# CPCLAB-UNIPI/MPC-code

Measured on AMD Instinct MI355X. Metric: closed-loop MPC steps/sec over batch, LMPC-CSTR N=50, higher is better.
Workload: dtype f64

## Files before the change

mpc-code_amd/csrc/mpc_amd.hip:

```cpp
#include "../../include/mpc_amd.h"
#include "mpc_device.hpp"
#include "mpc_tp.hpp"
#include "mpc_wave.hpp"
#include "mpc_soft.hpp"
#ifdef MPC_NL_PLANT_HEADER
#include MPC_NL_PLANT_HEADER
#endif

#include <hip/hip_runtime.h>
#include "mpc_comm.hpp"

#include <cmath>
#include <cstdint>
#include <cstdio>
#include <cstring>
#include <string>
#include <vector>

using namespace mpc;

#ifndef MPC_PART2
extern "C" const char *mpc_last_error(void) { return g_err; }
#endif

// ... 924 lines not shown
        X[j].put(X0);
    }
    MPC_STAMP_INIT
    int redo = 0;
    for (int k = 0; k < a.nsteps; k++) {
        unsigned bq = (unsigned)b;
        asm volatile("" : "+v"(bq));
        if (redo == 0) {
        if constexpr (RT::fits) {
            const int b16 = lane >> 4, r16 = lane & 15, b16c = b16 < NI ? b16 : 0;
            const unsigned bi = (unsigned)(blockIdx.x * NI + b16c);
            const bool inst16 = b16 < NI && (int)bi < a.B;
            double *const kq = keep + b16c * KEEP;
            if (inst16) {
                if (a.XP && r16 < NXP) (a.XP + (size_t)((size_t)k * NXP + r16) * Bs)[bi] = kq[KC::K_X + r16];
                if (a.XHAT && r16 < NX) (a.XHAT + (size_t)((size_t)k * NX + r16) * Bs)[bi] = kq[KC::K_XH + r16];
            }
            double xi_old = 0.0, xi_new = 0.0;
            if (P.estimator != MPC_EST_NONE)
                kalman_row16<NX, NY, ND, NXP, NU>(P, r16, b16 < NI, kq, KC::K_X, KC::K_XH, KC::K_P, a.pyp + k * NY, tab, T + b16c * RT::XCH, xi_old, xi_new);
            if (inst16 && a.DHAT && r16 >= NX && r16 < NE) (a.DHAT + (size_t)((size_t)k * ND + (r16 - NX)) * Bs)[bi] = xi_new;
            double delta = row16_max(r16 < NE ? fabs(xi_new - xi_old) : 0.0);
            __syncthreads();
            if (Cfg::RZ * NI * LD < 4 * RT::XCH) { for (int i = lane; i < NI * LD; i += 64) T[Cfg::RZ * NI * LD + i] = 0.0; }
            double dh[NDD], usv[NU];
            MPC_UNROLL for (int i = 0; i < ND; i++) dh[i] = kq[KC::K_DH + i];
            MPC_UNROLL for (int i = 0; i < NU; i++) usv[i] = kq[KC::K_US + i];
            int it_ss; double vrow;
            const int st_ss = target_row16<NX, NU, NY, ND, NGS, NHS>(P, r16, tab, a.usp + k * NU, a.ysp + k * NY, dh, usv, kq + KC::K_TW, twv + b16c, inst16, vrow, it_ss);
            const bool trow = r16 < NX + NU && b16 < NI;
            const double prev = trow ? kq[KC::K_XS + r16] : 0.0;
            const double tnew = (st_ss != kInfeasible && trow) ? vrow : prev;
            delta = dmax(delta, row16_max(fabs(tnew - prev)));
            if (trow) kq[KC::K_XS + r16] = tnew;
            if (inst16) {
                if (a.XS && r16 < NX) (a.XS + (size_t)((size_t)k * NX + r16) * Bs)[bi] = tnew;
                if (a.US && r16 >= NX && trow) (a.US + (size_t)((size_t)k * NU + (r16 - NX)) * Bs)[bi] = tnew;
                if (a.st_dyn && r16 == 0) { (a.st_ss + (size_t)k * Bs)[bi] = st_ss; (a.it_ss + (size_t)k * Bs)[bi] = it_ss; }
            }
            if (r16 == 0 && b16 < NI) outv[b16c * Cfg::OUT] = delta;
            __syncthreads();
        }
        if (valid) {
            double xh[NX], dh[NDD], u[NU], xs[NX], us[NU], delta = 0.0;
            MPC_UNROLL for (int i = 0; i < NX; i++) { xh[i] = kp[KC::K_XH + i]; xs[i] = kp[KC::K_XS + i]; }
            MPC_UNROLL for (int i = 0; i < ND; i++) dh[i] = kp[KC::K_DH + i];
            MPC_UNROLL for (int i = 0; i < NU; i++) { u[i] = kp[KC::K_U + i]; us[i] = kp[KC::K_US + i]; }
            if constexpr (RT::fits) delta = outv[lane * Cfg::OUT];
            else {
                double x[NXP];
                double xh_pred[NX], dh_prev[NDD], xs_prev[NX], us_prev[NU];
                MPC_UNROLL for (int i = 0; i < NXP; i++) x[i] = kp[KC::K_X + i];
                MPC_UNROLL for (int i = 0; i < NX; i++) { xh[i] = kp[KC::K_XH + i]; xs[i] = kp[KC::K_XS + i]; xh_pred[i] = xh[i]; xs_prev[i] = xs[i]; }
                MPC_UNROLL for (int i = 0; i < ND; i++) { dh[i] = kp[KC::K_DH + i]; dh_prev[i] = dh[i]; }
                MPC_UNROLL for (int i = 0; i < NU; i++) { u[i] = kp[KC::K_U + i]; us[i] = kp[KC::K_US + i]; us_prev[i] = us[i]; }
                if (a.XP) { MPC_UNROLL for (int i = 0; i < NXP; i++) (a.XP + (size_t)((size_t)k * NXP + i) * Bs)[bq] = x[i]; }
                if (a.XHAT) { MPC_UNROLL for (int i = 0; i < NX; i++) (a.XHAT + (size_t)((size_t)k * NX + i) * Bs)[bq] = xh[i]; }
                if (P.estimator != MPC_EST_NONE) {
                    double xi[NE], innov[NY];
                    MPC_UNROLL for (int i = 0; i < NX; i++) xi[i] = xh[i];
                    MPC_UNROLL for (int i = 0; i < ND; i++) xi[NX + i] = dh[i];
                    MPC_UNROLL for (int i = 0; i < NY; i++) {
                        double yh = P.fyc[i], yy = a.pyp[k * NY + i];
                        MPC_UNROLL for (int j = 0; j < NE; j++) yh += P.Ca[i][j] * xi[j];
// ... 32 lines not shown
            if (a.YS) {
                MPC_UNROLL for (int i = 0; i < NY; i++) {
                    double v = P.fyc[i];
                    MPC_UNROLL for (int j = 0; j < NX; j++) v += P.Cm[i][j] * xs[j];
                    MPC_UNROLL for (int j = 0; j < ND; j++) v += P.Cd[i][j] * dh[j];
                    (a.YS + (size_t)((size_t)k * NY + i) * Bs)[bq] = v;
                }
            }
            OcpInst<NS, NU> qi;
            build_inst<NX, NU, NY, ND, DU, NG>(P, xh, xs, us, dh, u, qi);
            const bool warm = wsv[lane] != 0 && delta <= kWsDelta && !P.no_warm;
            double *qd = q + lane * Cfg::QN;
            MPC_UNROLL for (int i = 0; i < NS; i++) { qd[i] = qi.z0[i]; qd[NS + i] = qi.zr[i]; qd[2 * NS + i] = qi.c[i]; qd[3 * NS + i] = qi.zlo_m[i]; qd[4 * NS + i] = qi.zhi_m[i]; qd[Cfg::QZN + i] = qi.zrN[i]; }
            MPC_UNROLL for (int i = 0; i < NU; i++) { qd[5 * NS + i] = qi.ur[i]; qd[5 * NS + NU + i] = qi.us[i]; }
            qd[5 * NS + 2 * NU] = delta;
            iflag[lane] = kWvValid | (qi.ok0 ? kWvOk0 : 0) | (warm ? kWvWarm : 0);
            itacc[lane] = 0;
            MPC_UNROLL for (int i = 0; i < NX; i++) { kp[KC::K_XH + i] = xh[i]; kp[KC::K_XS + i] = xs[i]; }
            MPC_UNROLL for (int i = 0; i < ND; i++) kp[KC::K_DH + i] = dh[i];
            MPC_UNROLL for (int i = 0; i < NU; i++) kp[KC::K_US + i] = us[i];
        } else if (lane < NI) iflag[lane] = 0;
        __syncthreads();
        }
        MPC_TSTAMP(0);
        wv_solve<NS, NU, DU, NC, MASKED, NI>(P, T, q, iflag, X, S, P.max_iter);
        MPC_STAMP_RESET
        if (lane == 0) {
            MPC_UNROLL for (int j = 0; j < NI; j++) {
                MPC_UNROLL for (int i = 0; i < NU; i++) outv[j * Cfg::OUT + i] = a_get(X[j].u[i]);
                MPC_UNROLL for (int i = 0; i < NS; i++) outv[j * Cfg::OUT + NU + i] = a_get(X[j].z[i]);
            }
        }
        if (P.term_cons && lane == P.N - 1) {
            MPC_UNROLL for (int j = 0; j < NI; j++) {
                double v = 0.0, c[NX];
                MPC_UNROLL for (int i = 0; i < NX; i++) { const double zr = q[j * Cfg::QN + NS + i]; c[i] = a_get(X[j].z[i]) - zr; v = dmax(v, fabs(c[i]) * frcp(dmax(1.0, fabs(zr)))); }
                outv[j * Cfg::OUT + NU + NS] = v;
                const int f = iflag[j];
                const bool again = redo < 2 && (f & kWvValid) && (f & kWvOk0) && S[j].status != kInfeasible && v > 1e-11 && v <= 1e-4;
                if (again) { MPC_UNROLL for (int i = 0; i < NX; i++) q[j * Cfg::QN + Cfg::QZN + i] -= c[i]; q[j * Cfg::QN + 5 * NS + 2 * NU] = v; }
                aimv[j] = again ? 1 : 0;
            }
        }
        __syncthreads();
        if (P.term_cons && redo < 2) {
            int any = 0;
            MPC_UNROLL for (int j = 0; j < NI; j++) any |= aimv[j];
// ... 1377 lines not shown
```

mpc-code_amd/csrc/mpc_tp.hpp:

```cpp
#pragma once
#include "mpc_device.hpp"

#ifdef MPC_STAMPS
#define MPC_TSTAMP(slot) do { const unsigned long long t_ = __builtin_amdgcn_s_memtime(); __builtin_amdgcn_s_waitcnt(0xC07F); \
    if (threadIdx.x == 0 && threadIdx.y == 0) mpc_stamp_buf[(blockIdx.x & 4095) * 8 + (slot)] += t_ - stamp_prev_; stamp_prev_ = t_; } while (0)
#else
#define MPC_TSTAMP(slot) do { } while (0)
#endif
#ifdef MPC_STAMPS_FINE
#define MPC_TSTAMP_IT(slot) MPC_TSTAMP(3)
#define MPC_TSTAMP_FINE(slot) MPC_TSTAMP(slot)
#else
#define MPC_TSTAMP_IT(slot) MPC_TSTAMP(slot)
#define MPC_TSTAMP_FINE(slot) do { } while (0)
#endif

namespace mpc {

template <int NS, int NU, int NC, int NW, int IPW, int XKEEP = 0>
struct TpCfg {
    static constexpr int NI = NW * IPW;
    static constexpr int NV = NS + NU, NKF = NU * NS, NLI = NU * (NU + 1) / 2;
    static constexpr int RA = 0, RA_SZ = (NC > NKF + NLI ? NC : NKF + NLI);
    static constexpr int RG = RA_SZ, RK = RG + NV, ROWS = RK + NU;
    static constexpr int LD = 65;
    static constexpr int T_DOUBLES = ROWS * NI * LD;
    static constexpr int QN = 5 * NS + 2 * NU + 1;
    static constexpr int ST_SL = 0, ST_SH = NC, ST_LL = 2 * NC, ST_LH = 3 * NC, ST_DV = 4 * NC, ST_U = 5 * NC, ST_Z = 5 * NC + NU, ROWS_ST = 5 * NC + NV;
    static constexpr int KEEP_MAX = 2 * NU + 3 * (NS + NU + 8) + XKEEP;
    static constexpr size_t lds_bytes() { return sizeof(double) * (T_DOUBLES + NI * QN + NI * 4 + NI * KEEP_MAX) + sizeof(int) * (4 * NI + 4); }
};

template <int CTRL, int ROW_MASK>
__device__ __forceinline__ double dpp_move(double old, double v)
{
    union { double d; int i[2]; } a, o, r; a.d = v; o.d = old;
    r.i[0] = __builtin_amdgcn_update_dpp(o.i[0], a.i[0], CTRL, ROW_MASK, 0xF, false);
// ... 622 lines not shown
```

mpc-code_amd/csrc/mpc_wave.hpp:

```cpp
#pragma once
#include "mpc_device.hpp"
#include "mpc_tp.hpp"

namespace mpc {

#ifdef MPC_WV_GENERIC_TILES
constexpr bool kWvGenericTiles = true;
#else
constexpr bool kWvGenericTiles = false;
#endif

template <int NS, int NU, int NC, int NI_>
struct WvCfg {
    static constexpr int NI = NI_;
    static constexpr int NV = NS + NU, NKF = NU * NS, NLI = NU * (NU + 1) / 2;
    static constexpr int RA = 0, RA_SZ = (NC > NKF + NLI ? NC : NKF + NLI);
    static constexpr int RG = RA_SZ, RK = RG + NV, RZ = RK + NU, ROWS = RZ + 1;
    __host__ __device__ static constexpr int ld(int N) { return (N + 1) | 1; }
    static constexpr int GUARD = 8;
    __host__ __device__ static constexpr int t_doubles(int N) { return GUARD + ROWS * NI * ld(N); }
    static constexpr int RL_A = ROWS, RL_B = RL_A + NS * NS, RL_C = RL_B + NS * NU, ROWS_LTV = RL_C + NS;
    __host__ __device__ static constexpr int t_doubles_ltv(int N) { return GUARD + ROWS_LTV * NI * ld(N); }
    static constexpr int QZN = 5 * NS + 2 * NU + 1;
    static constexpr int QN = QZN + NS;
// ... 20 lines not shown
    return u.d;
}
template <int NS, int NU, int NC>
struct WvIterA {
    AReg2 sl[NC], sh[NC], ll[NC], lh[NC], u[NU], z[NS];
    __device__ __forceinline__ void get(WvIter<NS, NU, NC> &X) const
    {
        MPC_UNROLL for (int i = 0; i < NC; i++) { X.sl[i] = a_get(sl[i]); X.sh[i] = a_get(sh[i]); X.ll[i] = a_get(ll[i]); X.lh[i] = a_get(lh[i]); }
        MPC_UNROLL for (int i = 0; i < NU; i++) X.u[i] = a_get(u[i]);
        MPC_UNROLL for (int i = 0; i < NS; i++) X.z[i] = a_get(z[i]);
    }
    __device__ __forceinline__ void put(const WvIter<NS, NU, NC> &X)
    {
        MPC_UNROLL for (int i = 0; i < NC; i++) { a_put(sl[i], X.sl[i]); a_put(sh[i], X.sh[i]); a_put(ll[i], X.ll[i]); a_put(lh[i], X.lh[i]); }
        MPC_UNROLL for (int i = 0; i < NU; i++) a_put(u[i], X.u[i]);
        MPC_UNROLL for (int i = 0; i < NS; i++) a_put(z[i], X.z[i]);
    }
};

struct WvInst { double mu, mu_sum, sm, inv_ncon, gscale, res_s, res_p; int stall, iters, status; bool on, warm, keep_u; };

enum : int { kWvOk0 = 1, kWvWarm = 2, kWvValid = 4, kWvKeepU = 8, kWvNoShift = 16 };

__device__ __forceinline__ double row16_sum(double v)
{
    v += dpp_move<0xB1, 0xF>(0.0, v);
    v += dpp_move<0x4E, 0xF>(0.0, v);
    v += dpp_move<0x141, 0xF>(0.0, v);
    v += dpp_move<0x140, 0xF>(0.0, v);
    return v;
}
__device__ __forceinline__ double row16_max(double v)
{
    v = dmax(v, dpp_move<0xB1, 0xF>(v, v));
    v = dmax(v, dpp_move<0x4E, 0xF>(v, v));
    v = dmax(v, dpp_move<0x141, 0xF>(v, v));
    v = dmax(v, dpp_move<0x140, 0xF>(v, v));
    return v;
}

template <int NS, int NU, bool HASM, int NC, bool MASKED, int NI, class PT, bool LTV = false, bool PAIR = false>
__device__ __forceinline__ void wv_solve(const PT &P, double *T, const double *q, const int *iflag,
                                         WvIterA<NS, NU, NC> (&X)[PAIR ? NI / 2 : NI], WvInst (&S)[PAIR ? NI / 2 : NI], int max_iter)
{
    static_assert(!LTV || (NS <= 4 && !HASM), "time-varying stage matrices: one 4 x 4 tile per state matrix, no cross term");
    using Cfg = WvCfg<NS, NU, NC, NI>;
    using Iter = WvIter<NS, NU, NC>;
    constexpr int NV = Cfg::NV, NKF = Cfg::NKF, NLI = Cfg::NLI, RA = Cfg::RA, RG = Cfg::RG, RK = Cfg::RK;
    static_assert(NS <= 8 && NU <= 2 && NI >= 1 && NI <= 4, "stage state <= 8 (2 x 2 tiles of 4 x 4), nu <= 2 (closed-form inverse of Lambda); at most four instances per product");
    static_assert(!PAIR || NI % 2 == 0, "pairs of instances");
    constexpr int NJ = PAIR ? NI / 2 : NI;
    const int lane = threadIdx.x, N = P.N, LD = Cfg::ld(N);
    const int k = PAIR ? (lane & 31) : lane;
    const int hsel = PAIR ? (lane >> 5) : 0;
    auto ji = [&](int j) -> int { return PAIR ? 2 * j + hsel : j; };
    const bool blk_on = k < N, last = k == N - 1;
    auto tk = [&](int row, int j) -> double & { return T[(row * NI + ji(j)) * LD + k]; };
    auto un = [](double v) -> double { return PAIR ? v : uni(v); };
    auto rsum = [](double v) -> double { return PAIR ? half_sum(v) : wave_sum(v); };
    auto rmax = [](double v) -> double { return PAIR ? half_max(v) : wave_max(v); };
    MPC_STAMP_INIT

    auto launder = [](const PT &Pin) -> const PT & { const PT *pp = &Pin; asm volatile("" : "+s"(pp)); return *pp; };
    struct Bnd { double lo[NC], hi[NC]; bool fl[NC], fh[NC]; };
    auto bounds = [&](const PT &Pl, int j, Bnd &Bd) {
        const double *qd = q + ji(j) * Cfg::QN;
        MPC_UNROLL for (int i = 0; i < NC; i++) {
            const double zlm = i >= NU ? qd[3 * NS + (i >= NU ? i - NU : 0)] : 0.0, zhm = i >= NU ? qd[4 * NS + (i >= NU ? i - NU : 0)] : 0.0;
            const double lm = i < NU ? Pl.ulo[i < NU ? i : 0] : zlm, hm = i < NU ? Pl.uhi[i < NU ? i : 0] : zhm;
            const double le = i < NU ? Pl.ulo[i < NU ? i : 0] : Pl.zlo_e[i >= NU ? i - NU : 0], he = i < NU ? Pl.uhi[i < NU ? i : 0] : Pl.zhi_e[i >= NU ? i - NU : 0];
            const double lo = last ? le : lm, hi = last ? he : hm;
            Bd.fl[i] = MASKED ? fin(lo) : true; Bd.fh[i] = MASKED ? fin(hi) : true;
            Bd.lo[i] = Bd.fl[i] ? lo : 0.0; Bd.hi[i] = Bd.fh[i] ? hi : 0.0;
        }
    };
    auto gradient = [&](const PT &Pl, int j, const Iter &Xj, double (&gu)[NU], double (&gz)[NS]) {
        const double *qd = q + ji(j) * Cfg::QN;
        double dz1[NS], du[NU];
        const double *qz = qd + (last ? Cfg::QZN : NS);
        MPC_UNROLL for (int i = 0; i < NS; i++) dz1[i] = Xj.z[i] - qz[i];
        MPC_UNROLL for (int i = 0; i < NU; i++) du[i] = Xj.u[i] - qd[5 * NS + i];
        MPC_UNROLL for (int i = 0; i < NS; i++) {
            double a = (NU + i < NC) ? Xj.lh[NU + i < NC ? NU + i : 0] - Xj.ll[NU + i < NC ? NU + i : 0] : 0.0;
// ... 14 lines not shown
        }
    };
    auto phase_a = [&](const PT &Pl, int j, WvInst &Sj, const Iter &Xj, int it) {
        Bnd Bd; bounds(Pl, j, Bd);
        double mu_p = 0.0, resp_p = 0.0, cres_p = 0.0, lmax_p = 0.0, hb[NC];
        MPC_UNROLL for (int i = 0; i < NC; i++) {
            const double v = i < NU ? Xj.u[i < NU ? i : 0] : Xj.z[i >= NU ? i - NU : 0];
            const double rh = Bd.fh[i] ? v + Xj.sh[i] - Bd.hi[i] : 0.0, rl = Bd.fl[i] ? v - Xj.sl[i] - Bd.lo[i] : 0.0;
            const double isl = frcp(Xj.sl[i]), ish = frcp(Xj.sh[i]);
            mu_p += Xj.sl[i] * Xj.ll[i] + Xj.sh[i] * Xj.lh[i];
            if (blk_on) tk(RA + i, j) = Xj.ll[i] * isl + Xj.lh[i] * ish;
            hb[i] = Xj.lh[i] * (rh * ish - 1.0) + Xj.ll[i] * (rl * isl + 1.0);
            resp_p = dmax(resp_p, dmax(fabs(rl), fabs(rh)));
            cres_p = dmax(cres_p, dmax(comp_measure(Xj.sl[i], Xj.ll[i]), comp_measure(Xj.sh[i], Xj.lh[i])));
            lmax_p = dmax(lmax_p, dmax(Xj.ll[i], Xj.lh[i]));
        }
        double gu[NU], gz[NS], pi[NS];
        gradient(Pl, j, Xj, gu, gz);
        if (blk_on) {
            MPC_UNROLL for (int i = 0; i < NU; i++) tk(RG + i, j) = gu[i] + hb[i];
            MPC_UNROLL for (int i = 0; i < NS; i++) tk(RG + NU + i, j) = gz[i] + (NU + i < NC ? hb[NU + i < NC ? NU + i : 0] : 0.0);
        }
        MPC_UNROLL for (int i = 0; i < NS; i++) pi[i] = blk_on ? gz[i] : 0.0;
        Sj.mu_sum = rsum(blk_on ? mu_p : 0.0);
        const double res_p = rmax(blk_on ? resp_p : 0.0), cres = rmax(blk_on ? cres_p : 0.0), lmax = rmax(blk_on ? lmax_p : 0.0);
        const bool ok_cp = (cres <= 1.0) && (res_p <= kTolFeas);
        double rs_p = 0.0;
        if (LTV) {
            if (it == 0 || ok_cp) {
                double An[NS][NS], g0[NS];
                const int kn = k + 1 < N ? k + 1 : (N > 0 ? N - 1 : 0);
                const bool upd = k + 1 < N;
                MPC_UNROLL for (int i = 0; i < NS; i++) { g0[i] = pi[i]; MPC_UNROLL for (int l = 0; l < NS; l++) { const double v = T[((Cfg::RL_A + i * NS + l) * NI + ji(j)) * LD + kn]; An[i][l] = upd ? v : 0.0; } }
                for (int s = N - 2; s >= 0; s--) {
                    double t[NS];
                    MPC_UNROLL for (int i = 0; i < NS; i++) { const double v = wave_dn1(pi[i], pi[i]); t[i] = (PAIR && !upd) ? 0.0 : v; }
                    MPC_UNROLL for (int i = 0; i < NS; i++) { double a = g0[i]; MPC_UNROLL for (int l = 0; l < NS; l++) a += An[l][i] * t[l]; pi[i] = a; }
                }
                MPC_UNROLL for (int i = 0; i < NU; i++) {
                    double a = gu[i];
                    MPC_UNROLL for (int l = 0; l < NS; l++) a += (blk_on ? tk(Cfg::RL_B + l * NU + i, j) : 0.0) * pi[l];
                    rs_p = dmax(rs_p, fabs(a));
                }
            }
        } else if (it == 0 || ok_cp) {
            MPC_UNROLL for (int e = 0; e < 6; e++) {
                const int d = 1 << e;
                if (d < N) {
// ... 30 lines not shown
        double ncon = 0.0;
        MPC_UNROLL for (int i = 0; i < NC; i++) {
            const double zlm = i >= NU ? un(qd[3 * NS + (i >= NU ? i - NU : 0)]) : 0.0, zhm = i >= NU ? un(qd[4 * NS + (i >= NU ? i - NU : 0)]) : 0.0;
            const double lm = i < NU ? Pl.ulo[i < NU ? i : 0] : zlm, hm = i < NU ? Pl.uhi[i < NU ? i : 0] : zhm;
            const double le = i < NU ? Pl.ulo[i < NU ? i : 0] : Pl.zlo_e[i >= NU ? i - NU : 0], he = i < NU ? Pl.uhi[i < NU ? i : 0] : Pl.zhi_e[i >= NU ? i - NU : 0];
            const bool flm = MASKED ? fin(lm) : true, fhm = MASKED ? fin(hm) : true, fle = MASKED ? fin(le) : true, fhe = MASKED ? fin(he) : true;
            ncon += (double)(N - 1) * ((flm ? 1 : 0) + (fhm ? 1 : 0)) + (fle ? 1 : 0) + (fhe ? 1 : 0);
        }
        Sj.inv_ncon = 1.0 / dmax(ncon, 1.0);
        if (Sj.on) {
            if (Sj.warm) {
                MPC_UNROLL for (int i = 0; i < NU; i++) Xj.u[i] = a_get(X[j].u[i]);
                MPC_UNROLL for (int i = 0; i < NC; i++) { Xj.ll[i] = a_get(X[j].ll[i]); Xj.lh[i] = a_get(X[j].lh[i]); }
            }
            const bool rep = k >= N - 1 || (myflag & kWvNoShift) != 0;
            double ll0[NC], lh0[NC];
            MPC_UNROLL for (int i = 0; i < NU; i++) {
                const double ulo = Pl.ulo[i], uhi = Pl.uhi[i];
                const bool f_lo = fin(ulo), f_hi = fin(uhi);
                double v;
                if (Sj.warm) {
                    const double t = wave_dn1(Xj.u[i], Xj.u[i]);
                    v = (rep || Sj.keep_u) ? Xj.u[i] : t;
                    if (f_lo) v = dmax(v, ulo);
                    if (f_hi) v = dmin(v, uhi);
                } else {
                    const double us = qd[5 * NS + NU + i];
                    double push;
                    if (f_lo && f_hi) push = 0.1 * (uhi - ulo);
                    else push = 0.1 * dmax(1.0, fabs(f_lo ? ulo : (f_hi ? uhi : 0.0)));
                    v = us;
                    if (f_lo) v = dmax(v, ulo + push);
                    if (f_hi) v = dmin(v, uhi - push);
                }
                Xj.u[i] = v;
            }
            MPC_UNROLL for (int i = 0; i < NC; i++) {
                if (Sj.warm) {
                    const double tl = wave_dn1(Xj.ll[i], Xj.ll[i]), th = wave_dn1(Xj.lh[i], Xj.lh[i]);
                    ll0[i] = rep ? Xj.ll[i] : tl; lh0[i] = rep ? Xj.lh[i] : th;
                } else { ll0[i] = 0.0; lh0[i] = 0.0; }
            }
            if (LTV) {
                double Ak[NS][NS], bk[NS], xk[NS];
                MPC_UNROLL for (int i = 0; i < NS; i++) {
                    double a = blk_on ? tk(Cfg::RL_C + i, j) : 0.0;
                    MPC_UNROLL for (int l = 0; l < NU; l++) a += (blk_on ? tk(Cfg::RL_B + i * NU + l, j) : 0.0) * Xj.u[l];
                    bk[i] = a;
// ... 7 lines not shown
                    double t[NS];
                    MPC_UNROLL for (int i = 0; i < NS; i++) { const double v = wave_up1(xk[i], xk[i]); t[i] = (PAIR && (k == 0 || !blk_on)) ? 0.0 : v; }
                    MPC_UNROLL for (int i = 0; i < NS; i++) { double a = bk[i]; MPC_UNROLL for (int l = 0; l < NS; l++) a += Ak[i][l] * t[l]; xk[i] = a; }
                }
                MPC_UNROLL for (int i = 0; i < NS; i++) Xj.z[i] = xk[i];
            } else {
                double xk[NS];
                MPC_UNROLL for (int i = 0; i < NS; i++) {
                    double a = qd[2 * NS + i];
                    MPC_UNROLL for (int l = 0; l < NU; l++) a += Pl.B[i][l] * Xj.u[l];
                    if (k == 0) { MPC_UNROLL for (int l = 0; l < NS; l++) a += Pl.A[i][l] * qd[l]; }
                    xk[i] = blk_on ? a : 0.0;
                }
                MPC_UNROLL for (int e = 0; e < 6; e++) {
                    const int d = 1 << e;
                    if (d < N) {
                        double t[NS];
                        MPC_UNROLL for (int i = 0; i < NS; i++) { const double v = e == 0 ? wave_up1(xk[i], xk[i]) : __shfl_up(xk[i], d, 64); t[i] = k >= d ? v : 0.0; }
                        MPC_UNROLL for (int i = 0; i < NS; i++) { double a = xk[i]; MPC_UNROLL for (int l = 0; l < NS; l++) a += Pl.Apow[e][i][l] * t[l]; xk[i] = a; }
                    }
                }
                MPC_UNROLL for (int i = 0; i < NS; i++) Xj.z[i] = xk[i];
            }
            Bnd Bd; bounds(Pl, j, Bd);
            const double ws_delta = un(qd[5 * NS + 2 * NU]);
            const double ws_smin = dmin(dmax(kWsKappa * ws_delta, kWsSMinLo), kWsSMinHi), ws_mu = kWsMuFactor * ws_smin * ws_smin;
            const double smin = Sj.warm ? ws_smin : kSMin;
            MPC_UNROLL for (int i = 0; i < NC; i++) {
                const double v = i < NU ? Xj.u[i < NU ? i : 0] : Xj.z[i >= NU ? i - NU : 0];
                Xj.sl[i] = Bd.fl[i] ? dmax(v - Bd.lo[i], smin) : 1.0; Xj.sh[i] = Bd.fh[i] ? dmax(Bd.hi[i] - v, smin) : 1.0;
                const double isl = frcp(Xj.sl[i]), ish = frcp(Xj.sh[i]);
                const double llo = Sj.warm ? dmax(ll0[i], ws_mu * isl) : kMu0 * isl, lhi = Sj.warm ? dmax(lh0[i], ws_mu * ish) : kMu0 * ish;
                Xj.ll[i] = Bd.fl[i] ? llo : 0.0; Xj.lh[i] = Bd.fh[i] ? lhi : 0.0;
            }
            X[j].put(Xj);
            phase_a(Pl, j, Sj, Xj, 0);
        }
        __builtin_amdgcn_sched_barrier(0);
    }

    MPC_TSTAMP(1);
    auto mm = [](double a, double b, double c) { return __builtin_amdgcn_mfma_f64_4x4x4f64(a, b, c, 0, 0, 0); };
    constexpr int RZ = Cfg::RZ;
    constexpr int SB = (NS + 3) / 4;
    constexpr bool VF = SB == 1 && !HASM && !kWvGenericTiles;
#define MPC_MM "v_mfma_f64_4x4x4_4b_f64 "
    struct TileCtx {
        int tr, tc; bool live;
        double *Tt, *trash;
        double Ar[SB][SB], Atr[SB][SB], Br[SB], Btr[SB];
        double *p_hu, *p_hz[SB], *p_kf, *p_k[SB], *p_kt[SB], *p_li;
        const double *p_a, *p_at, *p_b, *p_bt;
    };
    auto tile_ctx = [&](const PT &Pl) {
        int lo = threadIdx.x;
        asm volatile("" : "+v"(lo));
        TileCtx c;
        c.tr = lo >> 4; c.tc = lo & 3;
        const int tbq = (lo >> 2) & 3;
        c.live = tbq < NI;
        const int tb = c.live ? tbq : 0;
        const int tr = c.tr, tc = c.tc;
        c.Tt = T + tb * LD; c.trash = T - Cfg::GUARD;
        auto trow = [&](int row) -> double * { return c.Tt + (c.live ? row : RZ) * (NI * LD); };
// ... 337 lines not shown
            q_st[0][d] = st_u ? DU : DZn[0];
            MPC_UNROLL for (int i = 1; i < SB; i++) q_st[i][d] = DZn[i];
            MPC_UNROLL for (int i = 0; i < SB; i++) DZ[i] = DZn[i];
        };
        const int G = N / PD, rem = N - G * PD;
        for (int g = 0; g < G; g++) {
            MPC_UNROLL for (int d = 0; d < PD; d++) block(d, true);
            MPC_UNROLL for (int i = 0; i < SB; i++) { q_k[i] += PD; q_kt[i] += PD; q_st[i] += stp[i]; }
            q_kf += PD;
            if (LTV) { q_at += PD; q_bt += PD; }
        }
        MPC_UNROLL for (int d = 0; d < PD - 1; d++) { if (d < rem) block(d, false); }
    };

    AReg2 dvp[NJ][NC];
    for (int it = 0;; it++) {
        bool any_on = false;
        MPC_UNROLL for (int j = 0; j < NJ; j++) any_on = any_on || (PAIR ? __any(S[j].on) != 0 : S[j].on);
        if (!any_on) break;
        __syncthreads();
        pd_min = 1.0;
        tile_factor();
        __syncthreads();
        MPC_TSTAMP(2);
        tile_forward();
        __syncthreads();
        MPC_TSTAMP(3);
        {
            const unsigned long long bad = __ballot(((lane >> 2) & 3) < NI && !(pd_min > 0.0));
            MPC_UNROLL for (int j = 0; j < NJ; j++) {
                if (S[j].on && (bad & (0x000F000F000F000FULL << (4 * ji(j))))) { S[j].on = false; S[j].status = kInfeasible; S[j].iters = it; }
            }
        }
        MPC_UNROLL for (int j = 0; j < NJ; j++) {
            WvInst &Sj = S[j];
            if (Sj.on) {
                Iter Xj; X[j].get(Xj);
                const PT &Pl = P;
                Bnd Bd; bounds(Pl, j, Bd);
                double maff_p = 1.0, s1_p = 0.0, s2_p = 0.0, pl[NC], ph[NC], dvj[NC];
                MPC_UNROLL for (int i = 0; i < NC; i++) { dvj[i] = tk(RG + i, j); a_put(dvp[j][i], dvj[i]); }
                MPC_UNROLL for (int i = 0; i < NC; i++) {
                    const double v = i < NU ? Xj.u[i < NU ? i : 0] : Xj.z[i >= NU ? i - NU : 0];
                    const double isl = frcp(Xj.sl[i]), ish = frcp(Xj.sh[i]);
                    const double rh = Bd.fh[i] ? v + Xj.sh[i] - Bd.hi[i] : 0.0, rl = Bd.fl[i] ? v - Xj.sl[i] - Bd.lo[i] : 0.0;
                    const double dsh = Bd.fh[i] ? -rh - dvj[i] : 0.0, dsl = Bd.fl[i] ? rl + dvj[i] : 0.0;
                    const double qh = dsh * ish, ql = dsl * isl;
                    const double dlh = Bd.fh[i] ? -Xj.lh[i] - Xj.lh[i] * qh : 0.0, dll = Bd.fl[i] ? -Xj.ll[i] - Xj.ll[i] * ql : 0.0;
                    maff_p = dmax(maff_p, dmax(-ql, -qh));
                    if (Bd.fl[i]) maff_p = dmax(maff_p, 1.0 + ql);
                    if (Bd.fh[i]) maff_p = dmax(maff_p, 1.0 + qh);
                    s1_p += Xj.sl[i] * dll + Xj.ll[i] * dsl + Xj.sh[i] * dlh + Xj.lh[i] * dsh;
                    s2_p += dsl * dll + dsh * dlh;
                    pl[i] = dsl * dll; ph[i] = dsh * dlh;
                }
                const double m_aff = rmax(blk_on ? maff_p : 1.0), s1 = rsum(blk_on ? s1_p : 0.0), s2 = rsum(blk_on ? s2_p : 0.0);
                const double a_aff = frcp(m_aff);
                const double mu_aff = (Sj.mu_sum + a_aff * s1 + a_aff * a_aff * s2) * Sj.inv_ncon;
                const double rat = Sj.mu > 0.0 ? mu_aff * frcp(Sj.mu) : 0.0;
                Sj.sm = dmax(rat * rat * rat * Sj.mu, kMuFloor);
                double gu[NU], gz[NS], hc[NV];
                gradient(Pl, j, Xj, gu, gz);
                MPC_UNROLL for (int i = NC; i < NV; i++) hc[i] = 0.0;
                MPC_UNROLL for (int i = 0; i < NC; i++) {
                    const double v = i < NU ? Xj.u[i < NU ? i : 0] : Xj.z[i >= NU ? i - NU : 0];
                    const double isl = frcp(Xj.sl[i]), ish = frcp(Xj.sh[i]);
                    const double rh = Bd.fh[i] ? v + Xj.sh[i] - Bd.hi[i] : 0.0, rl = Bd.fl[i] ? v - Xj.sl[i] - Bd.lo[i] : 0.0;
                    const double rch = Bd.fh[i] ? Xj.sh[i] * Xj.lh[i] - dmax(Sj.sm, Xj.lh[i] * kSFloor) + ph[i] : 0.0;
                    const double rcl = Bd.fl[i] ? Xj.sl[i] * Xj.ll[i] - dmax(Sj.sm, Xj.ll[i] * kSFloor) + pl[i] : 0.0;
                    hc[i] = (-rch + Xj.lh[i] * rh) * ish + (rcl + Xj.ll[i] * rl) * isl;
                }
                if (blk_on) {
                    MPC_UNROLL for (int i = 0; i < NU; i++) tk(RG + i, j) = gu[i] + hc[i];
                    MPC_UNROLL for (int i = 0; i < NS; i++) tk(RG + NU + i, j) = gz[i] + hc[NU + i];
                }
            }
            __builtin_amdgcn_sched_barrier(0);
        }
        __syncthreads();
        MPC_TSTAMP(4);
        tile_rhs();
        __syncthreads();
        MPC_TSTAMP(5);
        tile_forward();
        __syncthreads();
        MPC_TSTAMP(3);
        MPC_UNROLL for (int j = 0; j < NJ; j++) {
            WvInst &Sj = S[j];
            if (Sj.on) {
                Iter Xj; X[j].get(Xj);
                const PT &Pl = P;
                Bnd Bd; bounds(Pl, j, Bd);
                double dvzj[NV], dvj[NC];
                MPC_UNROLL for (int i = 0; i < NC; i++) dvj[i] = a_get(dvp[j][i]);
                MPC_UNROLL for (int i = 0; i < NV; i++) dvzj[i] = tk(RG + i, j);
                double mcc_p = kTau;
                double dsl[NC], dsh[NC], dll[NC], dlh[NC];
                MPC_UNROLL for (int i = 0; i < NC; i++) {
                    const double v = i < NU ? Xj.u[i < NU ? i : 0] : Xj.z[i >= NU ? i - NU : 0];
                    const double isl = frcp(Xj.sl[i]), ish = frcp(Xj.sh[i]);
                    const double rh = Bd.fh[i] ? v + Xj.sh[i] - Bd.hi[i] : 0.0, rl = Bd.fl[i] ? v - Xj.sl[i] - Bd.lo[i] : 0.0;
                    const double ash = Bd.fh[i] ? -rh - dvj[i] : 0.0, asl = Bd.fl[i] ? rl + dvj[i] : 0.0;
                    const double alh = Bd.fh[i] ? -Xj.lh[i] - Xj.lh[i] * (ash * ish) : 0.0, all_ = Bd.fl[i] ? -Xj.ll[i] - Xj.ll[i] * (asl * isl) : 0.0;
                    const double rch = Bd.fh[i] ? Xj.sh[i] * Xj.lh[i] - dmax(Sj.sm, Xj.lh[i] * kSFloor) + ash * alh : 0.0;
                    const double rcl = Bd.fl[i] ? Xj.sl[i] * Xj.ll[i] - dmax(Sj.sm, Xj.ll[i] * kSFloor) + asl * all_ : 0.0;
                    dsh[i] = Bd.fh[i] ? -rh - dvzj[i] : 0.0; dsl[i] = Bd.fl[i] ? rl + dvzj[i] : 0.0;
                    dlh[i] = Bd.fh[i] ? (-rch - Xj.lh[i] * dsh[i]) * ish : 0.0; dll[i] = Bd.fl[i] ? (-rcl - Xj.ll[i] * dsl[i]) * isl : 0.0;
                    mcc_p = dmax(mcc_p, dmax(-dsl[i] * isl, -dsh[i] * ish));
                    if (Bd.fl[i]) mcc_p = dmax(mcc_p, -dll[i] * frcp_approx(Xj.ll[i]));
                    if (Bd.fh[i]) mcc_p = dmax(mcc_p, -dlh[i] * frcp_approx(Xj.lh[i]));
                }
                const double m_cc = rmax(blk_on ? mcc_p : kTau);
                const double alpha = m_cc <= kTau ? 1.0 : kTau * frcp(m_cc);
                MPC_UNROLL for (int i = 0; i < NC; i++) { Xj.sl[i] += alpha * dsl[i]; Xj.sh[i] += alpha * dsh[i]; Xj.ll[i] += alpha * dll[i]; Xj.lh[i] += alpha * dlh[i]; }
                MPC_UNROLL for (int i = 0; i < NU; i++) Xj.u[i] += alpha * dvzj[i];
                MPC_UNROLL for (int i = 0; i < NS; i++) Xj.z[i] += alpha * dvzj[NU + i];
                X[j].put(Xj);
                phase_a(Pl, j, Sj, Xj, it + 1);
            }
            __builtin_amdgcn_sched_barrier(0);
        }
        MPC_TSTAMP(6);
    }
}
#undef MPC_MM



template <int NX, int NU, int NY, int ND, int NGS = 0, int NHS = 0>
struct Row16Tab {
    static constexpr int NE = NX + ND, NR = NU - NHS, NCT = NX + NU + NY + NGS;
    static constexpr int E_A = 0, E_Q = NE, E_K = 2 * NE, E_DMIN = 2 * NE + NY, E_DMAX = E_DMIN + 1, ESZ = E_DMAX + 1;
    static constexpr int T_W = 0, T_LO = NR, T_HI = NR + 1, TSZ = NR + 2;
    static constexpr int DOUBLES = NE * ESZ + NCT * TSZ;
#ifdef MPC_ROW16_OFF
    static constexpr bool fits = false;
#else
    static constexpr bool fits = NE <= 16 && NCT <= 16;
#endif
    static constexpr int XCH = NE * NY + NE * NE;
};

template <int NX, int NU, int NY, int ND, int NGS = 0, int NHS = 0, class PT>
__device__ __forceinline__ void row16_fill_tables(const PT &P, double *tab, int lane)
{
// ... 44 lines not shown
        if (row) { MPC_UNROLL for (int j = 0; j < NY; j++) xch[r * NY + j] = PCt[j]; }
        __syncthreads();
        double all[NE][NY], S[NY][NY];
        MPC_UNROLL for (int l = 0; l < NE; l++) { MPC_UNROLL for (int j = 0; j < NY; j++) all[l][j] = xch[l * NY + j]; }
        MPC_UNROLL for (int i = 0; i < NY; i++) { MPC_UNROLL for (int j = 0; j < NY; j++) { double a = P.Rkf[i][j]; MPC_UNROLL for (int l = 0; l < NE; l++) a += P.Ca[i][l] * all[l][j]; S[i][j] = a; } }
        MPC_UNROLL for (int i = 0; i < NY; i++) { MPC_UNROLL for (int j = 0; j < i; j++) { const double a = 0.5 * (S[i][j] + S[j][i]); S[i][j] = a; S[j][i] = a; } }
        sym_inverse<NY>(S);
        MPC_UNROLL for (int j = 0; j < NY; j++) { double a = 0.0; MPC_UNROLL for (int l = 0; l < NY; l++) a += PCt[l] * S[l][j]; Kr[j] = a; }
        double Pc[NE], U[NE];
        MPC_UNROLL for (int j = 0; j < NE; j++) { double a = Pr[j]; MPC_UNROLL for (int m = 0; m < NY; m++) a -= Kr[m] * all[j][m]; Pc[j] = a; }
        MPC_UNROLL for (int j = 0; j < NE; j++) { double a = 0.0; MPC_UNROLL for (int l = 0; l < NE; l++) a += Pc[l] * P.Aa[j][l]; U[j] = a; }
        double *xu = xch + NE * NY;
        if (row) { MPC_UNROLL for (int j = 0; j < NE; j++) xu[r * NE + j] = U[j]; }
        __syncthreads();
        double Pn[NE];
        MPC_UNROLL for (int j = 0; j < NE; j++) Pn[j] = e[RT::E_Q + j];
        MPC_UNROLL for (int l = 0; l < NE; l++) { const double al = e[RT::E_A + l]; MPC_UNROLL for (int j = 0; j < NE; j++) Pn[j] += al * xu[l * NE + j]; }
        if (row) { MPC_UNROLL for (int j = 0; j < NE; j++) kp[p_off + r * NE + j] = Pn[j]; }
    } else {
        MPC_UNROLL for (int j = 0; j < NY; j++) Kr[j] = e[RT::E_K + j];
    }
    double v = xi_old;
    MPC_UNROLL for (int l = 0; l < NY; l++) v += Kr[l] * innov[l];
    if (P.has_dsat && r >= NX) v = dmin(dmax(v, e[RT::E_DMIN]), e[RT::E_DMAX]);
    xi_new = v;
    __syncthreads();
    if (row) kp[xi_off + r] = v;
}

template <int NX, int NU, int NY, int ND, int NGS = 0, int NHS = 0, class PT>
__device__ __forceinline__ int target_row16(const PT &P, int r, const double *tab, const double *usp, const double *ysp, const double *dh,
                                            const double *us_prev, double *tw, int *twv, bool inst_on, double &v_out, int &iters)
{
    using RT = Row16Tab<NX, NU, NY, ND, NGS, NHS>;
    constexpr int NV = NX + NU, NC = RT::NCT, NR = RT::NR, NE = RT::NE;
    const bool row = r < NC;
    const int rr = row ? r : 0;
    const double *t = tab + NE * RT::ESZ + rr * RT::TSZ;
    double Wr[NR];
    MPC_UNROLL for (int c = 0; c < NR; c++) Wr[c] = row ? t[RT::T_W + c] : 0.0;
    const double tlo = t[RT::T_LO], thi = t[RT::T_HI];
    const bool fl = row && fin(tlo), fh = row && fin(thi);
    const double lo = fl ? tlo : 0.0, hi = fh ? thi : 0.0;
    double cx[NX], e[NY], vp[NV], yp[NY], gr[NR], y[NR];
    MPC_UNROLL for (int i = 0; i < NX; i++) { double a = P.fxc[i]; MPC_UNROLL for (int j = 0; j < ND; j++) a += P.Bd[i][j] * dh[j]; cx[i] = a; }
    MPC_UNROLL for (int i = 0; i < NY; i++) { double a = P.fyc[i]; MPC_UNROLL for (int j = 0; j < ND; j++) a += P.Cd[i][j] * dh[j]; e[i] = a; }
    MPC_UNROLL for (int q = 0; q < NV; q++) { double a = 0.0; MPC_UNROLL for (int j = 0; j < NX; j++) a -= P.Ep[q][j] * cx[j]; vp[q] = a; }
// ... 27 lines not shown
    const double ncon = row16_sum((fl ? 1.0 : 0.0) + (fh ? 1.0 : 0.0));
    const double inv_ncon = 1.0 / dmax(ncon, 1.0);
    {
        double Hi[NR][NR];
        MPC_UNROLL for (int i = 0; i < NR; i++) { MPC_UNROLL for (int j = 0; j < NR; j++) Hi[i][j] = P.Hr[i][j]; }
        sym_inverse<NR>(Hi);
        MPC_UNROLL for (int i = 0; i < NR; i++) { double a = 0.0; MPC_UNROLL for (int j = 0; j < NR; j++) a += Hi[i][j] * gr[j]; y[i] = -a; }
    }
    double s_lo, s_hi, l_lo, l_hi;
    {
        double v = w0; MPC_UNROLL for (int c = 0; c < NR; c++) v += Wr[c] * y[c];
        s_lo = fl ? dmax(v - lo, kSMin) : 1.0; s_hi = fh ? dmax(hi - v, kSMin) : 1.0;
        l_lo = fl ? kMu0 * frcp(s_lo) : 0.0; l_hi = fh ? kMu0 * frcp(s_hi) : 0.0;
    }
    if (*twv != 0) {
        double dl = row ? fabs(w0 - tw[2 * NR + 2 * NC + rr]) : 0.0;
        MPC_UNROLL for (int c = 0; c < NR; c++) dl = dmax(dl, fabs(gr[c] - tw[NR + 2 * NC + c]));
        const double delta = row16_max(dl);
        if (delta <= kWsDelta) {
            const double smin = dmin(dmax(kWsKappa * delta, kWsSMinLo), kWsSMinHi), wmu = kWsMuFactor * smin * smin;
            MPC_UNROLL for (int c = 0; c < NR; c++) y[c] = tw[c];
            double v = w0; MPC_UNROLL for (int c = 0; c < NR; c++) v += Wr[c] * y[c];
            s_lo = fl ? dmax(v - lo, smin) : 1.0; s_hi = fh ? dmax(hi - v, smin) : 1.0;
            l_lo = fl ? dmax(tw[NR + rr], wmu * frcp(s_lo)) : 0.0; l_hi = fh ? dmax(tw[NR + NC + rr], wmu * frcp(s_hi)) : 0.0;
        }
    }
    double gscale = 1.0; int stall = 0, status = kMaxIter;
    MPC_UNROLL for (int c = 0; c < NR; c++) gscale = dmax(gscale, fabs(gr[c]));
    bool on = inst_on;
    iters = 0;
    for (int it = 0;; it++) {
        if (!__any(on ? 1 : 0)) break;
        double v = w0; MPC_UNROLL for (int c = 0; c < NR; c++) v += Wr[c] * y[c];
        const double r_lo = fl ? v - s_lo - lo : 0.0, r_hi = fh ? v + s_hi - hi : 0.0;
        const double is_lo = frcp(s_lo), is_hi = frcp(s_hi);
        const double sig = l_lo * is_lo + l_hi * is_hi;
        const double mu = row16_sum(s_lo * l_lo + s_hi * l_hi) * inv_ncon;
        const double res_p = row16_max(dmax(fabs(r_lo), fabs(r_hi)));
        const double cres = row16_max(dmax(comp_measure(s_lo, l_lo), comp_measure(s_hi, l_hi)));
        const double lmax = row16_max(dmax(l_lo, l_hi));
        double grad[NR], res_s = 0.0;
        MPC_UNROLL for (int c = 0; c < NR; c++) {
            double a = gr[c]; MPC_UNROLL for (int j = 0; j < NR; j++) a += P.Hr[c][j] * y[j];
            a += row16_sum((l_hi - l_lo) * Wr[c]);
            grad[c] = a; res_s = dmax(res_s, fabs(a));
        }
        if (on) {
            iters = it;
            const bool ok_cp = (cres <= 1.0) && (res_p <= kTolFeas);
            stall = ok_cp ? stall + 1 : 0;
            if (ok_cp && (res_s <= kTolStat * gscale || (stall > kStallMax && res_s <= kTolStatAcc * gscale))) { status = kSolved; on = false; }
            else if (lmax > kInfeasZ * gscale || !(fabs(mu) < 1.0e300)) { status = kInfeasible; on = false; }
            else if (it == P.max_iter) { status = kMaxIter; on = false; }
        }
        double Ht[NR][NR];
        MPC_UNROLL for (int i = 0; i < NR; i++) { MPC_UNROLL for (int j = 0; j <= i; j++) { const double a = P.Hr[i][j] + row16_sum(sig * Wr[i] * Wr[j]); Ht[i][j] = a; Ht[j][i] = a; } }
        const bool pd = sym_inverse<NR>(Ht);
        if (on && !pd) { status = kInfeasible; on = false; }
        double dy[NR], ds_lo = 0.0, ds_hi = 0.0, dl_lo = 0.0, dl_hi = 0.0, sm = 0.0, alpha = 1.0;
        MPC_UNROLL for (int pass = 0; pass < 2; pass++) {
            double rc_lo, rc_hi, rhs[NR];
            if (pass == 0) { rc_lo = fl ? s_lo * l_lo : 0.0; rc_hi = fh ? s_hi * l_hi : 0.0; }
            else {
                rc_lo = fl ? s_lo * l_lo - dmax(sm, l_lo * kSFloor) + ds_lo * dl_lo : 0.0;
                rc_hi = fh ? s_hi * l_hi - dmax(sm, l_hi * kSFloor) + ds_hi * dl_hi : 0.0;
            }
            const double h = (-rc_hi + l_hi * r_hi) * is_hi + (rc_lo + l_lo * r_lo) * is_lo;
            MPC_UNROLL for (int c = 0; c < NR; c++) rhs[c] = grad[c] + row16_sum(h * Wr[c]);
            MPC_UNROLL for (int i = 0; i < NR; i++) { double a = 0.0; MPC_UNROLL for (int j = 0; j < NR; j++) a += Ht[i][j] * rhs[j]; dy[i] = -a; }
            double dv = 0.0; MPC_UNROLL for (int c = 0; c < NR; c++) dv += Wr[c] * dy[c];
            ds_hi = fh ? -r_hi - dv : 0.0; ds_lo = fl ? r_lo + dv : 0.0;
            dl_hi = fh ? (-rc_hi - l_hi * ds_hi) * is_hi : 0.0;
            dl_lo = fl ? (-rc_lo - l_lo * ds_lo) * is_lo : 0.0;
            double m = dmax(pass == 0 ? 1.0 : kTau, dmax(-ds_lo * is_lo, -ds_hi * is_hi));
            if (fl) m = dmax(m, -dl_lo * frcp_approx(l_lo));
            if (fh) m = dmax(m, -dl_hi * frcp_approx(l_hi));
            m = row16_max(m);
// ... 25 lines not shown
```

Measured before the change: 33.50 million.

## Use raw v_max/v_min f64, batch wave reductions, early-exit target solver loop

Introduces inline-asm v_max_f64/v_min_f64 helpers and uses them in place of dmax/dmin in reductions and clamps, skipping the NaN-handling code the generic max/min may produce. Fuses several independent sum and max wave reductions into one interleaved DPP pass so their latencies overlap. Adds an early break in the steady-state target IPM loop once every row has converged, which avoids one extra Hessian inverse per solve. Also adds optional per-step timestamp macros for profiling. The raw asm changes NaN semantics and hides the operations from compiler scheduling.

```diff
diff --git a/mpc-code_amd/csrc/mpc_amd.hip b/mpc-code_amd/csrc/mpc_amd.hip
--- a/mpc-code_amd/csrc/mpc_amd.hip
+++ b/mpc-code_amd/csrc/mpc_amd.hip
@@ -970,6 +970,7 @@
             if (inst16 && a.DHAT && r16 >= NX && r16 < NE) (a.DHAT + (size_t)((size_t)k * ND + (r16 - NX)) * Bs)[bi] = xi_new;
             double delta = row16_max(r16 < NE ? fabs(xi_new - xi_old) : 0.0);
             __syncthreads();
+            MPC_TSTAMP_STEP(0);
             if (Cfg::RZ * NI * LD < 4 * RT::XCH) { for (int i = lane; i < NI * LD; i += 64) T[Cfg::RZ * NI * LD + i] = 0.0; }
             double dh[NDD], usv[NU];
             MPC_UNROLL for (int i = 0; i < ND; i++) dh[i] = kq[KC::K_DH + i];
@@ -979,7 +980,7 @@
             const bool trow = r16 < NX + NU && b16 < NI;
             const double prev = trow ? kq[KC::K_XS + r16] : 0.0;
             const double tnew = (st_ss != kInfeasible && trow) ? vrow : prev;
-            delta = dmax(delta, row16_max(fabs(tnew - prev)));
+            delta = vmax(delta, row16_max(fabs(tnew - prev)));
             if (trow) kq[KC::K_XS + r16] = tnew;
             if (inst16) {
                 if (a.XS && r16 < NX) (a.XS + (size_t)((size_t)k * NX + r16) * Bs)[bi] = tnew;
@@ -988,6 +989,7 @@
             }
             if (r16 == 0 && b16 < NI) outv[b16c * Cfg::OUT] = delta;
             __syncthreads();
+            MPC_TSTAMP_STEP(1);
         }
         if (valid) {
             double xh[NX], dh[NDD], u[NU], xs[NX], us[NU], delta = 0.0;
@@ -1066,7 +1068,7 @@
         } else if (lane < NI) iflag[lane] = 0;
         __syncthreads();
         }
-        MPC_TSTAMP(0);
+        MPC_TSTAMP_WV(0, 6);
         wv_solve<NS, NU, DU, NC, MASKED, NI>(P, T, q, iflag, X, S, P.max_iter);
         MPC_STAMP_RESET
         if (lane == 0) {
diff --git a/mpc-code_amd/csrc/mpc_tp.hpp b/mpc-code_amd/csrc/mpc_tp.hpp
--- a/mpc-code_amd/csrc/mpc_tp.hpp
+++ b/mpc-code_amd/csrc/mpc_tp.hpp
@@ -13,6 +13,13 @@
 #else
 #define MPC_TSTAMP_IT(slot) MPC_TSTAMP(slot)
 #define MPC_TSTAMP_FINE(slot) do { } while (0)
+#endif
+#ifdef MPC_STAMPS_STEP
+#define MPC_TSTAMP_WV(slot, step_slot) MPC_TSTAMP(step_slot)
+#define MPC_TSTAMP_STEP(step_slot) MPC_TSTAMP(step_slot)
+#else
+#define MPC_TSTAMP_WV(slot, step_slot) MPC_TSTAMP(slot)
+#define MPC_TSTAMP_STEP(step_slot) do { } while (0)
 #endif
 
 namespace mpc {
diff --git a/mpc-code_amd/csrc/mpc_wave.hpp b/mpc-code_amd/csrc/mpc_wave.hpp
--- a/mpc-code_amd/csrc/mpc_wave.hpp
+++ b/mpc-code_amd/csrc/mpc_wave.hpp
@@ -66,6 +66,71 @@
 
 enum : int { kWvOk0 = 1, kWvWarm = 2, kWvValid = 4, kWvKeepU = 8, kWvNoShift = 16 };
 
+__device__ __forceinline__ double vmax(double a, double b)
+{
+    if (__builtin_constant_p(a) || __builtin_constant_p(b)) return dmax(a, b);
+    double r;
+    asm("v_max_f64 %0, %1, %2" : "=v"(r) : "v"(a), "v"(b));
+    return r;
+}
+__device__ __forceinline__ double vmin(double a, double b)
+{
+    if (__builtin_constant_p(a) || __builtin_constant_p(b)) return dmin(a, b);
+    double r;
+    asm("v_min_f64 %0, %1, %2" : "=v"(r) : "v"(a), "v"(b));
+    return r;
+}
+__device__ __forceinline__ double wv_comp_measure(double s, double l)
+{
+    return dmin(vmin(s, l) * (1.0 / kTolC), s * l * (1.0 / kTolMu));
+}
+__device__ __forceinline__ double wv_wave_max(double v)
+{
+    v = vmax(v, dpp_move<0xB1, 0xF>(v, v));
+    v = vmax(v, dpp_move<0x4E, 0xF>(v, v));
+    v = vmax(v, dpp_move<0x141, 0xF>(v, v));
+    v = vmax(v, dpp_move<0x140, 0xF>(v, v));
+    v = vmax(v, dpp_move<0x142, 0xA>(v, v));
+    v = vmax(v, dpp_move<0x143, 0xC>(v, v));
+    return lane63(v);
+}
+__device__ __forceinline__ double wv_half_max(double v)
+{
+    v = vmax(v, dpp_move<0xB1, 0xF>(v, v));
+    v = vmax(v, dpp_move<0x4E, 0xF>(v, v));
+    v = vmax(v, dpp_move<0x141, 0xF>(v, v));
+    v = vmax(v, dpp_move<0x140, 0xF>(v, v));
+    v = vmax(v, dpp_move<0x142, 0xA>(v, v));
+    const double lo = lane_of(v, 31), hi = lane_of(v, 63);
+    return (threadIdx.x & 32) ? hi : lo;
+}
+template <bool PAIR, int NSUM, int NMAX>
+__device__ __forceinline__ void wv_reduce(double (&s)[NSUM], double (&m)[NMAX])
+{
+#define MPC_WV_RSTEP(CTRL, MASK) do { \
+        double ts_[NSUM], tm_[NMAX]; \
+        MPC_UNROLL for (int i = 0; i < NSUM; i++) ts_[i] = dpp_move<CTRL, MASK>(0.0, s[i]); \
+        MPC_UNROLL for (int i = 0; i < NMAX; i++) tm_[i] = dpp_move<CTRL, MASK>(m[i], m[i]); \
+        MPC_UNROLL for (int i = 0; i < NSUM; i++) s[i] += ts_[i]; \
+        MPC_UNROLL for (int i = 0; i < NMAX; i++) m[i] = vmax(m[i], tm_[i]); \
+    } while (0)
+    MPC_WV_RSTEP(0xB1, 0xF);
+    MPC_WV_RSTEP(0x4E, 0xF);
+    MPC_WV_RSTEP(0x141, 0xF);
+    MPC_WV_RSTEP(0x140, 0xF);
+    MPC_WV_RSTEP(0x142, 0xA);
+    if (!PAIR) MPC_WV_RSTEP(0x143, 0xC);
+#undef MPC_WV_RSTEP
+    if (PAIR) {
+        const bool up = (threadIdx.x & 32) != 0;
+        MPC_UNROLL for (int i = 0; i < NSUM; i++) { const double lo = lane_of(s[i], 31), hi = lane_of(s[i], 63); s[i] = up ? hi : lo; }
+        MPC_UNROLL for (int i = 0; i < NMAX; i++) { const double lo = lane_of(m[i], 31), hi = lane_of(m[i], 63); m[i] = up ? hi : lo; }
+    } else {
+        MPC_UNROLL for (int i = 0; i < NSUM; i++) s[i] = lane63(s[i]);
+        MPC_UNROLL for (int i = 0; i < NMAX; i++) m[i] = lane63(m[i]);
+    }
+}
+
 __device__ __forceinline__ double row16_sum(double v)
 {
     v += dpp_move<0xB1, 0xF>(0.0, v);
@@ -76,10 +141,10 @@
 }
 __device__ __forceinline__ double row16_max(double v)
 {
-    v = dmax(v, dpp_move<0xB1, 0xF>(v, v));
-    v = dmax(v, dpp_move<0x4E, 0xF>(v, v));
-    v = dmax(v, dpp_move<0x141, 0xF>(v, v));
-    v = dmax(v, dpp_move<0x140, 0xF>(v, v));
+    v = vmax(v, dpp_move<0xB1, 0xF>(v, v));
+    v = vmax(v, dpp_move<0x4E, 0xF>(v, v));
+    v = vmax(v, dpp_move<0x141, 0xF>(v, v));
+    v = vmax(v, dpp_move<0x140, 0xF>(v, v));
     return v;
 }
 
@@ -101,8 +166,7 @@
     const bool blk_on = k < N, last = k == N - 1;
     auto tk = [&](int row, int j) -> double & { return T[(row * NI + ji(j)) * LD + k]; };
     auto un = [](double v) -> double { return PAIR ? v : uni(v); };
-    auto rsum = [](double v) -> double { return PAIR ? half_sum(v) : wave_sum(v); };
-    auto rmax = [](double v) -> double { return PAIR ? half_max(v) : wave_max(v); };
+    auto rmax = [](double v) -> double { return PAIR ? wv_half_max(v) : wv_wave_max(v); };
     MPC_STAMP_INIT
 
     auto launder = [](const PT &Pin) -> const PT & { const PT *pp = &Pin; asm volatile("" : "+s"(pp)); return *pp; };
@@ -163,8 +227,10 @@
             MPC_UNROLL for (int i = 0; i < NS; i++) tk(RG + NU + i, j) = gz[i] + (NU + i < NC ? hb[NU + i < NC ? NU + i : 0] : 0.0);
         }
         MPC_UNROLL for (int i = 0; i < NS; i++) pi[i] = blk_on ? gz[i] : 0.0;
-        Sj.mu_sum = rsum(blk_on ? mu_p : 0.0);
-        const double res_p = rmax(blk_on ? resp_p : 0.0), cres = rmax(blk_on ? cres_p : 0.0), lmax = rmax(blk_on ? lmax_p : 0.0);
+        double rs[1] = { blk_on ? mu_p : 0.0 }, rm[3] = { blk_on ? resp_p : 0.0, blk_on ? cres_p : 0.0, blk_on ? lmax_p : 0.0 };
+        wv_reduce<PAIR>(rs, rm);
+        Sj.mu_sum = rs[0];
+        const double res_p = rm[0], cres = rm[1], lmax = rm[2];
         const bool ok_cp = (cres <= 1.0) && (res_p <= kTolFeas);
         double rs_p = 0.0;
         if (LTV) {
@@ -241,8 +307,8 @@
                 if (Sj.warm) {
                     const double t = wave_dn1(Xj.u[i], Xj.u[i]);
                     v = (rep || Sj.keep_u) ? Xj.u[i] : t;
-                    if (f_lo) v = dmax(v, ulo);
-                    if (f_hi) v = dmin(v, uhi);
+                    if (f_lo) v = vmax(v, ulo);
+                    if (f_hi) v = vmin(v, uhi);
                 } else {
                     const double us = qd[5 * NS + NU + i];
                     double push;
@@ -296,6 +362,7 @@
                 }
                 MPC_UNROLL for (int i = 0; i < NS; i++) Xj.z[i] = xk[i];
             }
+            MPC_TSTAMP_STEP(2);
             Bnd Bd; bounds(Pl, j, Bd);
             const double ws_delta = un(qd[5 * NS + 2 * NU]);
             const double ws_smin = dmin(dmax(kWsKappa * ws_delta, kWsSMinLo), kWsSMinHi), ws_mu = kWsMuFactor * ws_smin * ws_smin;
@@ -308,12 +375,14 @@
                 Xj.ll[i] = Bd.fl[i] ? llo : 0.0; Xj.lh[i] = Bd.fh[i] ? lhi : 0.0;
             }
             X[j].put(Xj);
+            MPC_TSTAMP_STEP(3);
             phase_a(Pl, j, Sj, Xj, 0);
+            MPC_TSTAMP_STEP(4);
         }
         __builtin_amdgcn_sched_barrier(0);
     }
 
-    MPC_TSTAMP(1);
+    MPC_TSTAMP_WV(1, 4);
     auto mm = [](double a, double b, double c) { return __builtin_amdgcn_mfma_f64_4x4x4f64(a, b, c, 0, 0, 0); };
     constexpr int RZ = Cfg::RZ;
     constexpr int SB = (NS + 3) / 4;
@@ -697,10 +766,10 @@
         pd_min = 1.0;
         tile_factor();
         __syncthreads();
-        MPC_TSTAMP(2);
+        MPC_TSTAMP_WV(2, 5);
         tile_forward();
         __syncthreads();
-        MPC_TSTAMP(3);
+        MPC_TSTAMP_WV(3, 5);
         {
             const unsigned long long bad = __ballot(((lane >> 2) & 3) < NI && !(pd_min > 0.0));
             MPC_UNROLL for (int j = 0; j < NJ; j++) {
@@ -729,7 +798,9 @@
                     s2_p += dsl * dll + dsh * dlh;
                     pl[i] = dsl * dll; ph[i] = dsh * dlh;
                 }
-                const double m_aff = rmax(blk_on ? maff_p : 1.0), s1 = rsum(blk_on ? s1_p : 0.0), s2 = rsum(blk_on ? s2_p : 0.0);
+                double rs[2] = { blk_on ? s1_p : 0.0, blk_on ? s2_p : 0.0 }, rm[1] = { blk_on ? maff_p : 1.0 };
+                wv_reduce<PAIR>(rs, rm);
+                const double m_aff = rm[0], s1 = rs[0], s2 = rs[1];
                 const double a_aff = frcp(m_aff);
                 const double mu_aff = (Sj.mu_sum + a_aff * s1 + a_aff * a_aff * s2) * Sj.inv_ncon;
                 const double rat = Sj.mu > 0.0 ? mu_aff * frcp(Sj.mu) : 0.0;
@@ -753,13 +824,13 @@
             __builtin_amdgcn_sched_barrier(0);
         }
         __syncthreads();
-        MPC_TSTAMP(4);
+        MPC_TSTAMP_WV(4, 5);
         tile_rhs();
         __syncthreads();
-        MPC_TSTAMP(5);
+        MPC_TSTAMP_WV(5, 5);
         tile_forward();
         __syncthreads();
-        MPC_TSTAMP(3);
+        MPC_TSTAMP_WV(3, 5);
         MPC_UNROLL for (int j = 0; j < NJ; j++) {
             WvInst &Sj = S[j];
             if (Sj.on) {
@@ -795,7 +866,7 @@
             }
             __builtin_amdgcn_sched_barrier(0);
         }
-        MPC_TSTAMP(6);
+        MPC_TSTAMP_WV(6, 5);
     }
 }
 #undef MPC_MM
@@ -886,7 +957,7 @@
     }
     double v = xi_old;
     MPC_UNROLL for (int l = 0; l < NY; l++) v += Kr[l] * innov[l];
-    if (P.has_dsat && r >= NX) v = dmin(dmax(v, e[RT::E_DMIN]), e[RT::E_DMAX]);
+    if (P.has_dsat && r >= NX) v = vmin(vmax(v, e[RT::E_DMIN]), e[RT::E_DMAX]);
     xi_new = v;
     __syncthreads();
     if (row) kp[xi_off + r] = v;
@@ -960,7 +1031,7 @@
             MPC_UNROLL for (int c = 0; c < NR; c++) y[c] = tw[c];
             double v = w0; MPC_UNROLL for (int c = 0; c < NR; c++) v += Wr[c] * y[c];
             s_lo = fl ? dmax(v - lo, smin) : 1.0; s_hi = fh ? dmax(hi - v, smin) : 1.0;
-            l_lo = fl ? dmax(tw[NR + rr], wmu * frcp(s_lo)) : 0.0; l_hi = fh ? dmax(tw[NR + NC + rr], wmu * frcp(s_hi)) : 0.0;
+            l_lo = fl ? vmax(tw[NR + rr], wmu * frcp(s_lo)) : 0.0; l_hi = fh ? vmax(tw[NR + NC + rr], wmu * frcp(s_hi)) : 0.0;
         }
     }
     double gscale = 1.0; int stall = 0, status = kMaxIter;
@@ -975,8 +1046,8 @@
         const double sig = l_lo * is_lo + l_hi * is_hi;
         const double mu = row16_sum(s_lo * l_lo + s_hi * l_hi) * inv_ncon;
         const double res_p = row16_max(dmax(fabs(r_lo), fabs(r_hi)));
-        const double cres = row16_max(dmax(comp_measure(s_lo, l_lo), comp_measure(s_hi, l_hi)));
-        const double lmax = row16_max(dmax(l_lo, l_hi));
+        const double cres = row16_max(vmax(wv_comp_measure(s_lo, l_lo), wv_comp_measure(s_hi, l_hi)));
+        const double lmax = row16_max(vmax(l_lo, l_hi));
         double grad[NR], res_s = 0.0;
         MPC_UNROLL for (int c = 0; c < NR; c++) {
             double a = gr[c]; MPC_UNROLL for (int j = 0; j < NR; j++) a += P.Hr[c][j] * y[j];
@@ -991,6 +1062,7 @@
             else if (lmax > kInfeasZ * gscale || !(fabs(mu) < 1.0e300)) { status = kInfeasible; on = false; }
             else if (it == P.max_iter) { status = kMaxIter; on = false; }
         }
+        if (!__any(on ? 1 : 0)) break;
         double Ht[NR][NR];
         MPC_UNROLL for (int i = 0; i < NR; i++) { MPC_UNROLL for (int j = 0; j <= i; j++) { const double a = P.Hr[i][j] + row16_sum(sig * Wr[i] * Wr[j]); Ht[i][j] = a; Ht[j][i] = a; } }
         const bool pd = sym_inverse<NR>(Ht);
```

Result: no change. 33.41 million (-0.3%).
